# DoubangoTelecom/compv

Measured on AMD Instinct MI355X. Metric: Mpixels/s Sobel->Canny->HoughSHT on 4K uint8, higher is better.
Workload: dtype u8; 1 GPU; batched 3840x2160 uint8 frames, Sobel3x3 -> Canny(59,119) -> HoughSHT(rho=1, theta=1deg, thr=100); 256 distinct frames resident per GPU as 8 batches of 32, a step processes one batch, steps rotate over the batches; frames_per_gpu=32, resident_batches=8, parallelism=frames sharded across 1 GPU(s), no data-path collective

## Files before the change

### compv_amd/csrc/api.cpp

```cpp
#include "api_internal.hpp"

namespace {
__attribute__((noinline, optnone)) float libmCosf(float x) { return cosf(x); }
__attribute__((noinline, optnone)) float libmSinf(float x) { return sinf(x); }

void gradientThresholds(float fLow, float fHigh, int* tLow, int* tHigh)
{
	const float l = fLow < 1.f ? 1.f : (fLow > 65535.f ? 65535.f : fLow);
	const float h = fHigh < 1.f ? 1.f : (fHigh > 65535.f ? 65535.f : fHigh);
	uint16_t lo = static_cast<uint16_t>(l), hi = static_cast<uint16_t>(h);
	lo = static_cast<uint16_t>(std::max<int>(1, lo));
	hi = static_cast<uint16_t>(std::max<int>(lo + 2, hi));
	*tLow = lo; *tHigh = hi;
}

void cannyCoverage(size_t W, int* simdEnd, int* cStart)
{
	const size_t maxCols = W - 1;
	size_t mpw = 1;
	if (maxCols >= 16) mpw = 16; else if (maxCols >= 8) mpw = 8;
	if (mpw == 1) { *simdEnd = 1; *cStart = 1; return; }
	size_t col = 1;
	while (col + (mpw - 1) < maxCols) col += mpw;
	*simdEnd = static_cast<int>(col);
// ... 550 lines not shown
	if (run.copyBack) HIPCHK(ctx, hipMemcpyAsync(run.copyBack, run.patchOut, bytes, hipMemcpyDeviceToDevice, st));
	p->bitsValid = true;
	return COMPVHIP_OK;
}

int compvhip_plan_canny(compvhip_plan* p, const uint8_t* d_in, float tLow, float tHigh, int ksize, int type, uint8_t* d_edges, void* stream)
{
	if (!p) return COMPVHIP_E_INVALID_PARAMETER;
	if (int rc = refuseBeyondLaunchLimit(p->ctx, p->frames, "compvhip_plan_canny")) return rc;
	StepRun run;
	return planCannyImpl(p, run, d_in, tLow, tHigh, ksize, type, d_edges, static_cast<hipStream_t>(stream), true);
}

int compvhip_api::pixfmtBytes(int fmt)
{
	if (fmt < COMPVHIP_FMT_RGBA32 || fmt > COMPVHIP_FMT_Y) return 0;
	return fmt <= COMPVHIP_FMT_BGRA32 ? 4 : (fmt <= COMPVHIP_FMT_BGR24 ? 3 : (fmt == COMPVHIP_FMT_Y ? 1 : 2));
}

int compvhip_api::checkPixfmt(compvhip_ctx* ctx, int fmt, size_t W)
{
	if (fmt > COMPVHIP_FMT_Y && fmt <= COMPVHIP_FMT_HSV) return fail(ctx, COMPVHIP_E_INVALID_PARAMETER, "a format of the colour conversion calls only (compvhip_convert_frames)");
	if (!pixfmtBytes(fmt)) return fail(ctx, COMPVHIP_E_NOT_IMPLEMENTED, "pixel format without a grayscale conversion");
	if ((fmt == COMPVHIP_FMT_YUYV422 || fmt == COMPVHIP_FMT_UYVY422) && (W & 1)) return fail(ctx, COMPVHIP_E_INVALID_PARAMETER, "packed 4:2:2 needs an even width");
	return COMPVHIP_OK;
}

int compvhip_plan_grayscale(compvhip_plan* p, const uint8_t* d_in, int pixfmt, uint8_t* d_gray, void* stream)
{
	if (!p) return COMPVHIP_E_INVALID_PARAMETER;
	compvhip_ctx* ctx = p->ctx;
	if (!d_in || !d_gray) return fail(ctx, COMPVHIP_E_INVALID_PARAMETER, "null frame pointer");
	const int rc = checkPixfmt(ctx, pixfmt, p->W);
	if (rc) return rc;
	HIPCHK(ctx, hipSetDevice(ctx->device));
	hipStream_t st = static_cast<hipStream_t>(stream);
	if (p->timing) timelineClear(p);
	GrayArgs a;
	a.in = d_in; a.out = d_gray; a.W = static_cast<int>(p->W); a.H = static_cast<int>(p->H); a.S = static_cast<int>(p->S); a.So = static_cast<int>(p->S);
	Stamp s(p, st, "gray_kernel");
	HIPCHK(ctx, launch_gray(a, pixfmt, static_cast<int>(p->frames), st));
	return COMPVHIP_OK;
}

int compvhip_plan_otsu(compvhip_plan* p, const uint8_t* d_gray, int32_t* d_thresholds, void* stream)
{
	if (!p) return COMPVHIP_E_INVALID_PARAMETER;
	compvhip_ctx* ctx = p->ctx;
	if (!d_gray || !d_thresholds) return fail(ctx, COMPVHIP_E_INVALID_PARAMETER, "null pointer");
	if (misaligned(3, d_thresholds)) return fail(ctx, COMPVHIP_E_INVALID_PARAMETER, "levels must be 4-byte aligned");
	HIPCHK(ctx, hipSetDevice(ctx->device));
	int rc = ensurePreproc(p);
	if (rc) return rc;
	hipStream_t st = static_cast<hipStream_t>(stream);
	if (p->timing) timelineClear(p);
	Stamp s(p, st, "otsu_kernels");
	HIPCHK(ctx, launch_otsu(d_gray, static_cast<int>(p->W), static_cast<int>(p->H), static_cast<int>(p->S), p->S * p->H, static_cast<int>(p->frames), 0.5f, 1.f,
	                        p->hist, d_thresholds, nullptr, st));
	return COMPVHIP_OK;
}

int compvhip_api::checkFxpKernel(compvhip_ctx* ctx, size_t W, size_t H, const uint16_t* vt, const uint16_t* hz, size_t k)
{
	if (!vt || !hz || !(k & 1) || W < k || H < k) return fail(ctx, COMPVHIP_E_INVALID_PARAMETER, "convolution kernel: null, even size or larger than the image");
	if (k < 3 || k > static_cast<size_t>(kFxpMaxTaps)) return fail(ctx, COMPVHIP_E_NOT_IMPLEMENTED, "fixed-point convolution supports kernel sizes 3..15");
	return COMPVHIP_OK;
}

int compvhip_plan_convlt1_fixedpoint(compvhip_plan* p, const uint8_t* d_in, const uint16_t* vtKern, const uint16_t* hzKern, size_t kernSize, uint8_t* d_out,
                                     void* stream)
{
	if (!p) return COMPVHIP_E_INVALID_PARAMETER;
	compvhip_ctx* ctx = p->ctx;
	if (!d_in || !d_out) return fail(ctx, COMPVHIP_E_INVALID_PARAMETER, "null frame pointer");
	int rc = refuseBeyondLaunchLimit(ctx, p->frames, "compvhip_plan_convlt1_fixedpoint");
	if (rc) return rc;
	rc = checkFxpKernel(ctx, p->W, p->H, vtKern, hzKern, kernSize);
	if (rc) return rc;
	HIPCHK(ctx, hipSetDevice(ctx->device));
	const size_t span = p->S * p->H * p->frames;
	const bool alias = overlaps(d_in, span, d_out, span);
	if (alias) HIPCHK(ctx, p->blurTmp.reserve(ctx, span));
	hipStream_t st = static_cast<hipStream_t>(stream);
	if (p->timing) timelineClear(p);
	Stamp s(p, st, "convlt_fxp_kernels");
	HIPCHK(ctx, launch_convlt_fxp(d_in, p->blurTmp, d_out, static_cast<int>(p->W), static_cast<int>(p->H), static_cast<int>(p->S), p->S * p->H,
	                              static_cast<int>(p->frames), vtKern, hzKern, static_cast<int>(kernSize), st));
	return COMPVHIP_OK;
}

int compvhip_plan_edge_dete(compvhip_plan* p, const uint8_t* d_in, int op, uint8_t* d_out, void* stream)
{
	if (!p) return COMPVHIP_E_INVALID_PARAMETER;
	compvhip_ctx* ctx = p->ctx;
	if (!d_in || !d_out) return fail(ctx, COMPVHIP_E_INVALID_PARAMETER, "null frame pointer");
	if (op != COMPVHIP_OP_SOBEL && op != COMPVHIP_OP_SCHARR && op != COMPVHIP_OP_PREWITT)
		return fail(ctx, COMPVHIP_E_INVALID_PARAMETER, "invalid detector id");
	const size_t bytes = p->S * p->H * p->frames;
	if (overlaps(d_in, bytes, d_out, bytes)) return fail(ctx, COMPVHIP_E_INVALID_PARAMETER, "d_in and d_out must not alias");
	HIPCHK(ctx, hipSetDevice(ctx->device));
	hipStream_t st = static_cast<hipStream_t>(stream);
	if (p->timing) timelineClear(p);
	EdgeDeteArgs a;
	a.in = d_in; a.out = d_out; a.gmax = p->sums;
	a.inFrameStride = p->S * p->H; a.outFrameStride = p->S * p->H;
	a.W = static_cast<int>(p->W); a.H = static_cast<int>(p->H); a.S = static_cast<int>(p->S); a.So = static_cast<int>(p->S);
	a.tilesX = p->tilesX; a.tilesY = p->tilesY;
	Stamp s(p, st, "edge_dete_kernels");
	HIPCHK(ctx, launch_edge_dete(a, op, static_cast<int>(p->frames), st));
	return COMPVHIP_OK;
}

int compvhip_api::planShtImpl(compvhip_plan* p, const uint8_t* d_edges, int threshold, int maxLines, compvhip_line* d_lines, size_t lineCap, int32_t* d_counts,
                              hipStream_t st, const ShtOpts& o)
{
	compvhip_ctx* ctx = p->ctx;
	if (threshold <= 0) return fail(ctx, COMPVHIP_E_INVALID_PARAMETER, "threshold must be > 0");
	if (misaligned(3, d_lines, d_counts)) return fail(ctx, COMPVHIP_E_INVALID_PARAMETER, "lines and counts must be 4-byte aligned");
	if (!d_edges && !p->bitsValid) return fail(ctx, COMPVHIP_E_INVALID_STATE, "no edge masks: run compvhip_plan_canny first or pass d_edges");
	HIPCHK(ctx, hipSetDevice(ctx->device));
	int rc = ensureSht(p);
	if (rc) return rc;
	rc = ensureLineCap(p, std::max(lineCap, kMinLineCap));
	if (rc) return rc;
	if (p->timing && o.clearTimeline) timelineClear(p);
	const int frames = static_cast<int>(p->frames);
	size_t sortN = o.sortN;
	if (d_edges) {
		Stamp s(p, st, "bytes_to_bits_kernel");
		HIPCHK(ctx, launch_bytes_to_bits(d_edges, static_cast<int>(p->W), static_cast<int>(p->H), static_cast<int>(p->S), p->S * p->H, p->ebits, p->wb,
		                                 p->bitsFrameStride, frames, st));
		p->bitsValid = false;
	}
	ShtArgs a = shtArgs(p, threshold);
	a.outCounts = d_counts;
	a.hostStep = o.hostSlot; a.stepFlags = p->flags;
	const size_t capAll = p->lineCap * p->frames;
	const bool deviceSort = p->deviceSort && !o.pairsOnly;
	if (sortN != kSortExact) sortN = std::min(sortN, capAll);
	a.sortN = (o.pairsOnly || deviceSort || sortN == kSortExact) ? 0 : sortN;
	if (!p->countersFresh) HIPCHK(ctx, hipMemsetAsync(p->counters, 0, sizeof(int) * p->nCounts, st));
	p->countersFresh = false;
	{ Stamp s(p, st, "sht_compact_kernel"); HIPCHK(ctx, launch_sht_compact_tiles(a, p->vt, frames, st)); }
	{ Stamp s(p, st, "sht_vote_kernel"); HIPCHK(ctx, launch_sht_vote_tiles(a, p->vt, frames, st)); }
	{ Stamp s(p, st, "sht_reduce_kernel"); HIPCHK(ctx, launch_sht_reduce_tiles(a, p->vt, frames, st)); }
	{ Stamp s(p, st, "sht_lines_kernel"); HIPCHK(ctx, launch_sht_lines(a, frames, st)); }
	if (o.pairsOnly) {
		return COMPVHIP_OK;
	}
	if (deviceSort) {
		if (d_lines && lineCap) {
			Stamp s(p, st, "sht_sort_lines");
			ShtSortArgs q;
			q.sortedKeys = p->keysB; q.sortedVals = p->valsB; q.chunkHist = p->chunkHist; q.strengthStart = p->strengthStart; q.chunks = p->sortChunks;
			HIPCHK(ctx, launch_sht_sort_lines(a, q, frames, p->thetaStep, maxLines, d_lines, lineCap, st));
		}
		return COMPVHIP_OK;
	}
	if (sortN == kSortExact) {
		HIPCHK(ctx, hipMemcpyAsync(p->hTotals, p->lineTotal, sizeof(unsigned int), hipMemcpyDeviceToHost, st));
		HIPCHK(ctx, hipStreamSynchronize(st));
		sortN = std::min(static_cast<size_t>(p->hTotals[0]), capAll);
	}
	if (sortN) {
		Stamp s(p, st, "sht_sort_lines");
		size_t tb = p->sortTempBytes;
		hipError_t e = sht_sort_pairs(p->sortTemp, tb, p->keysA, p->keysB, p->valsA, p->valsB, sortN, p->keyBits, st);
		if (e != hipSuccess) return fail(ctx, COMPVHIP_E_HIP, "radix sort", e);
	}
	if (d_lines && lineCap) {
		Stamp s(p, st, "sht_decode_kernel");
		HIPCHK(ctx, launch_sht_decode(p->keysB, p->valsB, p->lineCounts, p->lineCap, frames, static_cast<int>(p->T), static_cast<int>(p->W + p->H), p->thetaStep, maxLines,
		                              p->strengthBits, d_lines, lineCap, st));
	}
	return COMPVHIP_OK;
}

int compvhip_plan_houghsht(compvhip_plan* p, const uint8_t* d_edges, int threshold, int maxLines, compvhip_line* d_lines, size_t lineCap,
                           int32_t* d_counts, void* stream)
{
	if (!p) return COMPVHIP_E_INVALID_PARAMETER;
	if (int rc = refuseBeyondLaunchLimit(p->ctx, p->frames, "compvhip_plan_houghsht")) return rc;
	return planShtImpl(p, d_edges, threshold, maxLines, d_lines, lineCap, d_counts, static_cast<hipStream_t>(stream), ShtOpts());
}

static int checkStep(compvhip_plan* p, const StepParams& sp)
{
	compvhip_ctx* ctx = p->ctx;
	int rc = refuseBeyondLaunchLimit(ctx, p->frames, "compvhip_plan_pipeline");
	if (rc) return rc;
	if (!sp.d_in || !sp.d_edges) return fail(ctx, COMPVHIP_E_INVALID_PARAMETER, "null frame pointer");
	rc = checkPixfmt(ctx, sp.pixfmt, p->W);
	if (rc) return rc;
	if (sp.d_cart && (!sp.d_lines || !sp.d_counts)) return fail(ctx, COMPVHIP_E_INVALID_PARAMETER, "toCartesian needs the line and count buffers");
	if (misaligned(3, sp.d_lines, sp.d_counts, sp.d_otsu, sp.d_cart)) return fail(ctx, COMPVHIP_E_INVALID_PARAMETER, "lines, counts, levels and endpoints must be 4-byte aligned");
	return COMPVHIP_OK;
}

static int enqueueStep(compvhip_plan* p, StepRun& run, const StepParams& sp, hipStream_t st, bool clearTimeline)
{
	compvhip_ctx* ctx = p->ctx;
	HIPCHK(ctx, hipSetDevice(ctx->device));
	const uint8_t* luma = sp.d_in;
	if (sp.pixfmt != COMPVHIP_FMT_Y) {
		uint8_t* gray = sp.d_gray;
		if (!gray) {
			HIPCHK(ctx, p->grayTmp.reserve(ctx, p->S * p->H * p->frames));
			gray = p->grayTmp;
		}
		if (p->timing && clearTimeline) timelineClear(p);
		clearTimeline = false;
		GrayArgs a;
		a.in = sp.d_in; a.out = gray; a.W = static_cast<int>(p->W); a.H = static_cast<int>(p->H); a.S = static_cast<int>(p->S); a.So = static_cast<int>(p->S);
		Stamp s(p, st, "gray_kernel");
		HIPCHK(ctx, launch_gray(a, sp.pixfmt, static_cast<int>(p->frames), st));
		luma = gray;
	}
	int rc = planCannyImpl(p, run, luma, sp.tLow, sp.tHigh, sp.ksize, sp.thresholdType, sp.d_edges, st, false, clearTimeline);
	if (rc) return rc;
	if (sp.d_otsu && sp.thresholdType == COMPVHIP_CANNY_THRESHOLD_OTSU)
		HIPCHK(ctx, hipMemcpyAsync(sp.d_otsu, p->otsu, sizeof(int32_t) * p->frames, hipMemcpyDeviceToDevice, st));
	return COMPVHIP_OK;
}

static int toCartesianImpl(compvhip_plan* p, const compvhip_line* d_lines, const int32_t* d_counts, size_t lineCap, int maxLines, float* d_cart, void* stream);

static int enqueueStepTail(compvhip_plan* p, const StepRun& run, const StepParams& sp, hipStream_t st, size_t sortN)
{
	ShtOpts o;
	o.clearTimeline = false; o.sortN = sortN; o.hostSlot = run.hostSlot;
	int rc = planShtImpl(p, nullptr, sp.threshold, sp.maxLines, sp.d_lines, sp.lineCap, sp.d_counts, st, o);
	if (rc) return rc;
	if (sp.d_cart) {
		rc = toCartesianImpl(p, sp.d_lines, sp.d_counts, sp.lineCap, sp.maxLines, sp.d_cart, st);
		if (rc) return rc;
	}
	return COMPVHIP_OK;
}

static int runStepSync(compvhip_plan* p, const StepParams& sp, hipStream_t st)
{
	StepRun run;
	int rc = enqueueStep(p, run, sp, st, true);
	if (rc) return rc;
	const size_t bytes = p->S * p->H * p->frames;
	for (;;) {
		rc = enqueueStepTail(p, run, sp, st, kSortExact);
		if (rc) return rc;
		bool done = false;
		rc = resolveConverged(p, run, st, &done);
		if (rc) return rc;
		if (done) break;
		do {
			rc = enqueueResolve(p, run, kSpecRounds, st);
			if (rc) return rc;
			rc = resolveConverged(p, run, st, &done);
			if (rc) return rc;
		} while (!done);
		if (run.copyBack) HIPCHK(p->ctx, hipMemcpyAsync(run.copyBack, run.patchOut, bytes, hipMemcpyDeviceToDevice, st));
	}
	return COMPVHIP_OK;
}

static int runStepAsync(compvhip_plan* p, const StepParams& sp, hipStream_t st, int* ticket)
{
	compvhip_ctx* ctx = p->ctx;
	*ticket = -1;
	int slot = -1;
	for (int i = 0; i < kAsyncDepth; ++i) if (!p->steps[i].used) { slot = i; break; }
	if (slot < 0) return fail(ctx, COMPVHIP_E_INVALID_STATE, "too many steps in flight: call compvhip_plan_wait first");
	const size_t bytes = p->S * p->H * p->frames;
	const size_t inBytes = bytes * static_cast<size_t>(sp.pixfmt == COMPVHIP_FMT_Y ? 1 : pixfmtBytes(sp.pixfmt));
	if (overlaps(sp.d_in, inBytes, sp.d_edges, bytes))
		return fail(ctx, COMPVHIP_E_INVALID_PARAMETER, "the asynchronous step needs distinct input and edge buffers");
	compvhip_plan::AsyncStep& stp = p->steps[slot];
	HIPCHK(ctx, hipSetDevice(ctx->device));
	if (!stp.done) HIPCHK(ctx, hipEventCreateWithFlags(&stp.done, hipEventDisableTiming));
	if (p->timeline.size() > kMaxTimeline) timelineClear(p);
	int* slotHost = p->hRounds + kSlotStride * slot;
	slotHost[kSlotTotal] = ~0;
	for (int i = 0; i < 4; ++i) slotHost[kSlotFlags + i] = 1;
	StepRun run;
	run.hostSlot = p->hRoundsDev + kSlotStride * slot;
	int rc = enqueueStep(p, run, sp, st, false);
	if (rc) return rc;
	rc = ensureSht(p);
	if (rc) return rc;
	rc = ensureLineCap(p, std::max(sp.lineCap, kMinLineCap));
	if (rc) return rc;
	const size_t capAll = p->lineCap * p->frames;
	const size_t sortN = p->deviceSort ? capAll : asyncSortRange(p->recentTotals, capAll);
	static_assert(kMaxRounds >= 4 && kSpecRounds <= 4, "the round flags compvhip_plan_wait looks at");
	if (run.roundsUsed > 4) return fail(ctx, COMPVHIP_E_INVALID_STATE, "more speculative rounds than flags the step reports");
	rc = enqueueStepTail(p, run, sp, st, sortN);
	if (rc) return rc;
	HIPCHK(ctx, hipEventRecord(stp.done, st));
	stp.used = true; stp.replay = false; stp.seq = ++p->stepSeq; stp.stream = st; stp.sp = sp; stp.sortN = sortN; stp.rounds = run.roundsUsed;
	*ticket = slot;
	return COMPVHIP_OK;
}

static StepParams classicStep(const uint8_t* d_in, float tLow, float tHigh, int threshold, int maxLines, uint8_t* d_edges, compvhip_line* d_lines, size_t lineCap,
                              int32_t* d_counts)
{
	StepParams sp;
	sp.d_in = d_in; sp.tLow = tLow; sp.tHigh = tHigh; sp.threshold = threshold; sp.maxLines = maxLines; sp.d_edges = d_edges; sp.d_lines = d_lines;
	sp.lineCap = lineCap; sp.d_counts = d_counts;
// ... 115 lines not shown
```

### compv_amd/csrc/kernels.hpp

```cpp
#pragma once
#include <hip/hip_runtime.h>
#include <stddef.h>
#include <stdint.h>

#include "../../include/compv_hip.h"

namespace compvhip {

#ifndef COMPVHIP_BAND_H
#define COMPVHIP_BAND_H 64
#endif
constexpr int kBandH = COMPVHIP_BAND_H;
#ifndef COMPVHIP_BAND_WORDS
#define COMPVHIP_BAND_WORDS 64
#endif
constexpr int kBandWords = COMPVHIP_BAND_WORDS;
constexpr int kResolveThreads = 512;
constexpr int kFrameSlot = 32;
constexpr int kResolveRows = kBandH * kBandWords / kResolveThreads;

struct CannyArgs {
	const uint8_t* in;
	uint8_t* out;
	uint32_t* ebits;
	uint32_t* ubits;
	const int2* thrDev;
	size_t inFrameStride, outFrameStride, bitsFrameStride;
	int W, H, S, So;
	int wb;
	int tilesX, tilesY;
	int tLow, tHigh;
	int simdEnd, cStart;
	int blockRows, groups;
	int ksize;
	int* zero; int nZero;
};

struct ResolveArgs {
	uint32_t* ebits;
	uint32_t* ubits;
	uint8_t* out;
	int* flags;
	uint8_t* dirty;
	size_t outFrameStride, bitsFrameStride;
	int H, So, wb;
	int round;
};

hipError_t launch_canny_tiles(const CannyArgs& a, int frames, bool gap, hipStream_t stream);
hipError_t launch_canny_tiles_swar(const CannyArgs& a, int frames, bool gap, hipStream_t stream);
hipError_t launch_canny_resolve(const ResolveArgs& a, int frames, hipStream_t stream);
size_t canny_resolve_dirty_bytes(int H, int wb, int frames);
hipError_t launch_mean_thresholds(const uint8_t* in, int W, int H, int S, size_t frameStride, int frames, float fLow, float fHigh,
                                  unsigned int* sums, int2* thr, hipStream_t stream);

struct EdgeDeteArgs {
	const uint8_t* in;
	uint8_t* out;
	unsigned int* gmax;
	size_t inFrameStride, outFrameStride;
	int W, H, S, So;
	int tilesX, tilesY;
	int blockRows, groups;
};
hipError_t launch_edge_dete(const EdgeDeteArgs& a, int op, int frames, hipStream_t stream);

struct ConvertArgs {
	const uint8_t* in[3];
	uint8_t* out[3];
	size_t inRow[3], inFrame[3], outRow[3], outFrame[3];
	int W, H;
};
hipError_t launch_convert(const ConvertArgs& a, int inFmt, int outFmt, int frames, hipStream_t stream);

struct GrayArgs {
	const uint8_t* in;
	uint8_t* out;
	int W, H, S, So;
};
hipError_t launch_gray(const GrayArgs& a, int fmt, int frames, hipStream_t stream);
constexpr int kOtsuMaxChunks = 128;
hipError_t launch_otsu(const uint8_t* in, int W, int H, int S, size_t frameStride, int frames, float fLowFactor, float fHighFactor, uint32_t* hist,
                       int32_t* otsu, void* thr, hipStream_t stream);

constexpr int kFxpMaxTaps = 15;
struct FxpArgs {
	const uint8_t* in;
	uint8_t* out;
	size_t inFrameStride, outFrameStride;
	int W, H, S, So;
	uint32_t kern[kFxpMaxTaps];
};
hipError_t launch_convlt_fxp(const uint8_t* in, uint8_t* tmp, uint8_t* out, int W, int H, int S, size_t frameStride, int frames, const uint16_t* vtKern,
                             const uint16_t* hzKern, int K, hipStream_t stream);

struct I16Args {
	const void* in;
	int16_t* out;
	int W, H, S, So, K;
	int kern[kFxpMaxTaps];
};
hipError_t launch_convlt_i16(const void* in, bool inIsU8, int16_t* tmp, int16_t* out, int W, int H, int S, int So, const int16_t* vtKern, const int16_t* hzKern,
                             int K, hipStream_t stream);

struct ShtArgs {
	const uint32_t* ebits;
	uint32_t* edges;
	int* edgeCounts;
	uint16_t* acc;
	const int32_t* sinQ;
	const int32_t* cosQ;
	uint32_t* lineKeys;
	uint32_t* lineVals;
	uint8_t* nmsFlags;
	int nmsRows;
	int* blockCounts;
	int lineBlocks;
	const int2* nmsRange;
	int nmsGroups;
	int* lineCounts;
	const int* stepFlags;
	int* hostStep;
	int32_t* outCounts;
	int* frameTotals;
	unsigned int* lineTotal;
	size_t sortN;
	size_t bitsFrameStride, edgeCap, accFrameStride, lineCap;
	int W, H, wb;
	int R, T, accPitch, barrier;
	int threshold, nmsLastCol;
	int frames;
	int strengthBits;
};
struct ShtTileArgs {
	const int32_t* kt;
	const int32_t* rowBase;
	uint8_t* partLo;
	uint8_t* partHi;
	uint8_t* colFlag;
	const int2* reach;
	int* tileCounts;
	int nx, ny, TW, TH, tiles;
	int Rw, rwPitch;
	int Tpad, groups;
	size_t tileCap;
};
constexpr int kShtMaxWindow = 1264;
hipError_t launch_sht_compact_tiles(const ShtArgs& a, const ShtTileArgs& v, int frames, hipStream_t stream);
hipError_t launch_sht_vote_tiles(const ShtArgs& a, const ShtTileArgs& v, int frames, hipStream_t stream);
hipError_t launch_sht_reduce_tiles(const ShtArgs& a, const ShtTileArgs& v, int frames, hipStream_t stream);
hipError_t launch_bytes_to_bits(const uint8_t* edges, int W, int H, int S, size_t frameStride, uint32_t* ebits, int wb, size_t bitsFrameStride,
                                int frames, hipStream_t stream);
hipError_t launch_sht_lines(const ShtArgs& a, int frames, hipStream_t stream);
hipError_t launch_sht_decode(const uint32_t* keys, const uint32_t* vals, const int* counts, size_t lineCap, int frames, int T, int barrier, float thetaStep,
                             int maxLines, int strengthBits, void* lines , size_t outCap, hipStream_t stream);
int sht_nms_groups(int T);
size_t sht_nms_rows(int R);
int sht_lines_blocks(int R);
hipError_t launch_sht_cartesian(const void* lines , const int* counts, size_t lineCap, int maxLines, int frames, int T, const float* cosT,
                                const float* invSinT, float thetaStep, float widthF, float r, float* out , hipStream_t stream);
hipError_t launch_sht_acc_transpose(const uint16_t* accT, int R, int T, int accPitch, int32_t* out, size_t outStride, hipStream_t stream);
constexpr int kShtSortChunk = 4096;
constexpr int kShtSortMaxStrengthBits = 13;
constexpr int kShtSortMaxChunks = 32;
struct ShtSortArgs {
	uint32_t* sortedKeys;
	uint32_t* sortedVals;
	uint16_t* chunkHist;
	uint32_t* strengthStart;
	int chunks;
};
hipError_t launch_sht_sort_lines(const ShtArgs& a, const ShtSortArgs& q, int frames, float thetaStep, int maxLines, void* lines , size_t outCap,
                                 hipStream_t stream);
hipError_t sht_sort_pairs(void* temp, size_t& tempBytes, const uint32_t* keysIn, uint32_t* keysOut, const uint32_t* valsIn, uint32_t* valsOut, size_t n,
                          int keyBits, hipStream_t stream);

struct ShtLineSetArgs {
	const uint32_t* ebits;
	const uint8_t* edges;
	size_t bitsFrameStride, edgeFrameStride;
	int wb, S;
	const int32_t* sinQ;
	const int32_t* cosQ;
	const compvhip_line* lines;
	const int32_t* lineCounts;
	size_t lineCap;
	int nLines;
	int W, H, R, T, barrier;
};
struct ShtSegArgs : ShtLineSetArgs {
	int minLength, maxGap;
	int32_t* perLine;
	compvhip_segment* segs;
	size_t segCap;
	int32_t* segCounts;
	int frame0;
};
hipError_t launch_sht_segments(const ShtSegArgs& a, int frames, int phase, hipStream_t stream);

struct ShtFitArgs : ShtLineSetArgs {
	int halfWidth;
	const compvhip_segment* segs;
	const int32_t* segCounts;
	size_t segCap;
	compvhip_line_fit* fits;
	size_t fitCap;
	int32_t* fitCounts;
	compvhip_line* refined;
	int frame0;
};
static_assert(sizeof(ShtLineSetArgs) == 104 && sizeof(ShtSegArgs) == 152 && sizeof(ShtFitArgs) == 176, "kernel argument layout");
hipError_t launch_sht_fit(const ShtFitArgs& a, int frames, hipStream_t stream);

struct CompArgs {
	const uint32_t* bits;
	size_t bitsFrameStride;
	int wb;
	int W, H;
	int words;
	uint32_t lastMask;
	int conn8;
	int minPixels;
	int32_t* parent;
	size_t parentFrameStride;
	int ps;
	int wantLabels;
	compvhip_component* comps;
	size_t compCap;
	int32_t* compCounts;
	int32_t* rowCounts;
	int frame0;
};
hipError_t launch_components(const CompArgs& a, int frames, int phase, hipStream_t stream);

struct ThreshArgs {
	const uint8_t* in;
	uint8_t* out;
	const int32_t* levels;
	size_t frameStride;
	int W, H, S;
	int t8;
};
hipError_t launch_threshold(const ThreshArgs& a, int frames, hipStream_t stream);
struct AdaptArgs {
	const uint8_t* in;
	uint8_t* out;
	size_t frameStride;
	int W, H, S;
	int r;
	uint32_t k;
	int delta, maxVal, invert;
};
hipError_t launch_threshold_adaptive(const AdaptArgs& a, int frames, hipStream_t stream);
constexpr int kMorphMaxStrel = 31;
constexpr size_t kMorphGeneralMaxMembers = 15;
enum { kMorphGeneral = 0, kMorphRect = 1, kMorphCross = 2 };
struct MorphArgs {
	const uint8_t* in;
	uint8_t* out;
	size_t frameStride;
	int W, H, S;
	int sw, sh;
	int dilate;
	int replicate;
	int kind;
	uint32_t rows[kMorphMaxStrel];
};
hipError_t launch_morph(const MorphArgs& a, int frames, hipStream_t stream);

struct FastArgs {
	const uint8_t* in;
	uint8_t* scores;
	size_t frameStride;
	int W, H, S;
	int t, N, nonmax;
	int maxFeatures;
	int* rowCounts;
	int* rowOffsets;
	int* hist;
	int* minScore;
	compvhip_corner* corners; size_t cornerCap;
	int32_t* counts;
};
hipError_t launch_fast(const FastArgs& a, int frames, int stage, hipStream_t stream);

constexpr int kMatchQueryBlock = 256;
constexpr int kMatchTrainSlice = 128;
constexpr int kMatchMaxKnn = 8;
constexpr int kMatchMaxDwords = 32;
struct MatchSliceArgs {
	const uint8_t* query;
	const uint8_t* train;
	const int32_t* queryCounts; const int32_t* trainCounts;
	int queryCap, trainCap, queryStride, trainStride;
	int queryShared, trainShared;
	int descDwords;
	int knn;
	int slices;
	uint32_t* partial;
	compvhip_match* matches;
};
hipError_t launch_match_slices(const MatchSliceArgs& a, int pairs, hipStream_t stream);
hipError_t launch_match_merge(const MatchSliceArgs& a, int pairs, hipStream_t stream);
hipError_t launch_match_reference(const MatchSliceArgs& a, int pairs, hipStream_t stream);
struct MatchGoodArgs {
	const compvhip_match* matches;
	const compvhip_match* reverse;
	const int32_t* queryCounts; const int32_t* trainCounts;
	int queryCap, trainCap, trainShared, knn;
	double ratio; int maxDistance, crossCheck;
	compvhip_match* good; size_t goodCap;
	int32_t* counts;
};
hipError_t launch_match_good(const MatchGoodArgs& a, int pairs, hipStream_t stream);

constexpr int kHomographySolveBlock = 64;
constexpr int kHomographyScoreBlock = 256;
struct HomographyPointsArgs {
	const compvhip_match* good; int goodCap;
	const int32_t* goodCounts;
// ... 232 lines not shown
```

### compv_amd/csrc/sht_sort_kernels.hip

```cpp
#include "device.hpp"

#include <type_traits>

namespace compvhip {

namespace {

constexpr int kChunk = kShtSortChunk;
constexpr int kSortThreads = 1024;
constexpr int kBins = 1 << kShtSortMaxStrengthBits;
static_assert(kChunk == 4096 && kBins == 8192, "key layout: 13 bits of inverted strength above 12 bits of chunk position");

}

__global__ __launch_bounds__(kSortThreads) void sht_chunk_sort_kernel(ShtArgs a, ShtSortArgs q)
{
	__shared__ uint32_t s_key[kChunk];
	__shared__ uint32_t s_hist[kBins];
	__shared__ uint32_t s_cnt[kSortThreads], s_wsum[kSortThreads / 64];
	__shared__ unsigned long long s_part[kSortThreads / 64];
	const int frame = blockIdx.y, chunk = blockIdx.x, t = threadIdx.x;
	const size_t nf = min((size_t)max(a.lineCounts[frame], 0), a.lineCap);
	const size_t c0 = (size_t)chunk * kChunk;
	if (c0 >= nf) return;
	const int m = (int)min((size_t)kChunk, nf - c0);
	const size_t base = dense_frame_base<kSortThreads>(a.lineCounts, frame, a.lineCap, s_part) + c0;
	const uint32_t mask = (1u << a.strengthBits) - 1u;
	const uint32_t* __restrict__ kin = a.lineKeys + base;
	const uint32_t* __restrict__ vin = a.lineVals + base;
	uint32_t e[4];
	{
		uint32_t kraw[4];
#pragma unroll
		for (int u = 0; u < 4; ++u) kraw[u] = kin[min(u * kSortThreads + t, m - 1)];
		asm volatile("" : "+v"(kraw[0]), "+v"(kraw[1]), "+v"(kraw[2]), "+v"(kraw[3]));
#pragma unroll
		for (int u = 0; u < 4; ++u) {
			const int i = u * kSortThreads + t;
			e[u] = i < m ? (((mask - (kraw[u] & mask)) << 12) | (uint32_t)i) : 0xffffffffu;
		}
	}
#pragma unroll
	for (int u = 0; u < kBins / kSortThreads; ++u) s_hist[t + u * kSortThreads] = 0u;
	const int lane = t & 63, wave = t >> 6;
	auto radix_pass = [&](auto nbits, int shift) {
		constexpr int NB = decltype(nbits)::value, BINS = 1 << NB;
		s_cnt[t] = 0u;
		__syncthreads();
		uint32_t rank[4], slot[4];
#pragma unroll
		for (int u = 0; u < 4; ++u) {
			const uint32_t d = (e[u] >> shift) & (uint32_t)(BINS - 1);
			uint64_t same = ~0ull;
#pragma unroll
			for (int b = 0; b < NB; ++b) {
				const bool bit = (d >> b) & 1u;
				const uint64_t bal = __ballot(bit);
				same &= bit ? bal : ~bal;
			}
			rank[u] = __builtin_amdgcn_mbcnt_hi((uint32_t)(same >> 32), __builtin_amdgcn_mbcnt_lo((uint32_t)same, 0u));
			slot[u] = (d * 4u + (uint32_t)u) * (uint32_t)(kSortThreads / 64) + (uint32_t)wave;
			if (rank[u] == 0u) s_cnt[slot[u]] = (uint32_t)__popcll(same);
		}
		__syncthreads();
		const uint32_t c = s_cnt[t];
		const uint32_t incl = wave_incl_scan(c, lane);
		if (lane == 63) s_wsum[wave] = incl;
		__syncthreads();
		uint32_t before = 0;
#pragma unroll
		for (int w = 0; w < kSortThreads / 64; ++w) before += (w < wave) ? s_wsum[w] : 0u;
		s_cnt[t] = before + incl - c;
		__syncthreads();
#pragma unroll
		for (int u = 0; u < 4; ++u) s_key[s_cnt[slot[u]] + rank[u]] = e[u];
		__syncthreads();
#pragma unroll
		for (int u = 0; u < 4; ++u) e[u] = s_key[u * kSortThreads + t];
	};
	radix_pass(std::integral_constant<int, 4>{}, 12);
	radix_pass(std::integral_constant<int, 3>{}, 16);
	radix_pass(std::integral_constant<int, 3>{}, 19);
	radix_pass(std::integral_constant<int, 3>{}, 22);
	uint32_t* __restrict__ kout = q.sortedKeys + base;
	uint32_t* __restrict__ vout = q.sortedVals + base;
	{
		uint32_t kk[4]; int lo[4], hi[4];
#pragma unroll
		for (int u = 0; u < 4; ++u) { const int i = min(t + u * kSortThreads, m - 1); kk[u] = s_key[i]; lo[u] = 0; hi[u] = i; }
#pragma unroll
		for (int s = 0; s < 12; ++s) {
#pragma unroll
			for (int u = 0; u < 4; ++u) {
				const int mid = (lo[u] + hi[u]) >> 1;
				const bool ge = s_key[mid] >= (kk[u] & ~4095u);
				hi[u] = ge ? mid : hi[u];
				lo[u] = ge ? lo[u] : mid + 1;
			}
		}
		uint32_t cell[4];
#pragma unroll
		for (int u = 0; u < 4; ++u) cell[u] = vin[kk[u] & 4095u];
		asm volatile("" : "+v"(cell[0]), "+v"(cell[1]), "+v"(cell[2]), "+v"(cell[3]));
#pragma unroll
		for (int u = 0; u < 4; ++u) {
			const int i = t + u * kSortThreads;
			if (i < m) {
				kout[i] = (kk[u] & ~4095u) | (uint32_t)(i - lo[u]);
				vout[i] = cell[u];
				atomicAdd(&s_hist[kk[u] >> 12], 1u);
			}
		}
	}
	__syncthreads();
	uint4* __restrict__ hout = reinterpret_cast<uint4*>(q.chunkHist + ((size_t)frame * q.chunks + chunk) * kBins);
	{
		const uint32_t* h = s_hist + 8 * t;
		hout[t] = make_uint4(h[0] | (h[1] << 16), h[2] | (h[3] << 16), h[4] | (h[5] << 16), h[6] | (h[7] << 16));
	}
}

__global__ __launch_bounds__(kSortThreads) void sht_strength_scan_kernel(ShtArgs a, ShtSortArgs q)
{
	__shared__ uint32_t s_wave[kSortThreads / 64];
	const int frame = blockIdx.x, t = threadIdx.x;
	const size_t nf = min((size_t)max(a.lineCounts[frame], 0), a.lineCap);
	if (nf == 0) return;
	const int nch = (int)((nf + kChunk - 1) / kChunk);
	uint32_t tot[8] = { 0, 0, 0, 0, 0, 0, 0, 0 };
	const uint4* __restrict__ h = reinterpret_cast<const uint4*>(q.chunkHist + (size_t)frame * q.chunks * kBins) + t;
	auto add8 = [](uint32_t (&d)[8], const uint4& v) {
		d[0] += v.x & 0xffffu; d[1] += v.x >> 16; d[2] += v.y & 0xffffu; d[3] += v.y >> 16;
		d[4] += v.z & 0xffffu; d[5] += v.z >> 16; d[6] += v.w & 0xffffu; d[7] += v.w >> 16;
	};
	const uint4 zero4 = make_uint4(0u, 0u, 0u, 0u);
	for (int c0 = 0; c0 < nch; c0 += 4) {
		uint4 v[4];
#pragma unroll
		for (int u = 0; u < 4; ++u) v[u] = h[(size_t)min(c0 + u, nch - 1) * (kBins / 8)];
#pragma unroll
		for (int u = 0; u < 4; ++u) add8(tot, (c0 + u < nch) ? v[u] : zero4);
	}
	uint32_t sum = 0;
#pragma unroll
	for (int u = 0; u < 8; ++u) { const uint32_t c = tot[u]; tot[u] = sum; sum += c; }
	uint32_t incl = sum;
	const int lane = t & 63, wave = t >> 6;
#pragma unroll
	for (int o = 1; o < 64; o <<= 1) {
		const uint32_t n = __shfl_up(incl, o);
		if (lane >= o) incl += n;
	}
	if (lane == 63) s_wave[wave] = incl;
	__syncthreads();
	uint32_t before = 0;
#pragma unroll
	for (int w = 0; w < kSortThreads / 64; ++w) before += (w < wave) ? s_wave[w] : 0u;
	const uint32_t excl = before + incl - sum;
	uint4* __restrict__ out = reinterpret_cast<uint4*>(q.strengthStart + (size_t)frame * kBins) + 2 * t;
	out[0] = make_uint4(excl + tot[0], excl + tot[1], excl + tot[2], excl + tot[3]);
	out[1] = make_uint4(excl + tot[4], excl + tot[5], excl + tot[6], excl + tot[7]);
}

__global__ __launch_bounds__(256) void sht_place_lines_kernel(ShtArgs a, ShtSortArgs q, float thetaStep, int maxLines, compvhip_line* __restrict__ lines, size_t outCap)
{
	__shared__ unsigned long long s_part[4];
	const int frame = blockIdx.y;
	const size_t nf = min((size_t)max(a.lineCounts[frame], 0), a.lineCap);
	const size_t i0 = (size_t)blockIdx.x * 256;
	if (i0 >= nf) return;
	const size_t base = dense_frame_base<256>(a.lineCounts, frame, a.lineCap, s_part);
	const size_t i = i0 + threadIdx.x;
	if (i >= nf) return;
	size_t limit = nf;
	if (maxLines > 0 && limit > (size_t)maxLines) limit = (size_t)maxLines;
	if (limit > outCap) limit = outCap;
	const uint32_t kv = q.sortedKeys[base + i];
	const uint32_t inv = kv >> 12, rank = kv & 4095u;
	const int c = (int)(i >> 12);
	size_t pos = (size_t)q.strengthStart[(size_t)frame * kBins + inv] + rank;
	const uint16_t* __restrict__ h = q.chunkHist + (size_t)frame * q.chunks * kBins + inv;
	for (int c0 = 0; c0 < c; c0 += 4) {
		uint32_t v[4];
#pragma unroll
		for (int u = 0; u < 4; ++u) v[u] = h[(size_t)min(c0 + u, c) * kBins];
#pragma unroll
		for (int u = 0; u < 4; ++u) pos += (c0 + u < c) ? v[u] : 0u;
	}
	if (pos >= limit) return;
	const uint32_t cell = q.sortedVals[base + i];
	const int row = (int)(cell / (uint32_t)a.T), col = (int)(cell - (uint32_t)row * (uint32_t)a.T);
	compvhip_line o;
	o.rho = (float)(a.barrier - row);
	o.theta = __fmul_rn((float)col, thetaStep);
	o.strength = (int32_t)(((1u << a.strengthBits) - 1u) - inv);
	o.row = row; o.col = col;
	lines[(size_t)frame * outCap + pos] = o;
}

hipError_t launch_sht_sort_lines(const ShtArgs& a, const ShtSortArgs& q, int frames, float thetaStep, int maxLines, void* lines, size_t outCap, hipStream_t stream)
{
	if (!lines || !outCap) return hipSuccess;
	hipLaunchKernelGGL(sht_chunk_sort_kernel, dim3((unsigned)q.chunks, (unsigned)frames), dim3(kSortThreads), 0, stream, a, q);
	hipLaunchKernelGGL(sht_strength_scan_kernel, dim3((unsigned)frames), dim3(kSortThreads), 0, stream, a, q);
	hipLaunchKernelGGL(sht_place_lines_kernel, dim3((unsigned)(q.chunks * (kChunk / 256)), (unsigned)frames), dim3(256), 0, stream, a, q, thetaStep, maxLines,
	                   reinterpret_cast<compvhip_line*>(lines), outCap);
	return hipGetLastError();
}

}
```

Baseline: 426,700 Mpixels/s.

## Replace per-chunk radix sort with stable ballot-based rank counting

The per-chunk LDS radix sort (four passes plus a binary search and a value gather) becomes a ranking kernel. Each wave groups lanes that share a strength via bit ballots, and waves commit packed u16 counters to LDS in turn order, which gives each line a stable rank within its strength. The placement kernel then reads values straight from the unsorted input. Chunk size doubles to 8192 and the LDS counter footprint scales with strengthBits. This removes the sorted-values buffer and most of the shuffling work, at the cost of serialising the waves' commits.

```diff
diff --git a/compv_amd/csrc/api.cpp b/compv_amd/csrc/api.cpp
--- a/compv_amd/csrc/api.cpp
+++ b/compv_amd/csrc/api.cpp
@@ -726,7 +726,7 @@
 		if (d_lines && lineCap) {
 			Stamp s(p, st, "sht_sort_lines");
 			ShtSortArgs q;
-			q.sortedKeys = p->keysB; q.sortedVals = p->valsB; q.chunkHist = p->chunkHist; q.strengthStart = p->strengthStart; q.chunks = p->sortChunks;
+			q.rankKeys = p->keysB; q.chunkHist = p->chunkHist; q.strengthStart = p->strengthStart; q.chunks = p->sortChunks;
 			HIPCHK(ctx, launch_sht_sort_lines(a, q, frames, p->thetaStep, maxLines, d_lines, lineCap, st));
 		}
 		return COMPVHIP_OK;
diff --git a/compv_amd/csrc/kernels.hpp b/compv_amd/csrc/kernels.hpp
--- a/compv_amd/csrc/kernels.hpp
+++ b/compv_amd/csrc/kernels.hpp
@@ -160,12 +160,11 @@
 hipError_t launch_sht_cartesian(const void* lines , const int* counts, size_t lineCap, int maxLines, int frames, int T, const float* cosT,
                                 const float* invSinT, float thetaStep, float widthF, float r, float* out , hipStream_t stream);
 hipError_t launch_sht_acc_transpose(const uint16_t* accT, int R, int T, int accPitch, int32_t* out, size_t outStride, hipStream_t stream);
-constexpr int kShtSortChunk = 4096;
+constexpr int kShtSortChunk = 8192;
 constexpr int kShtSortMaxStrengthBits = 13;
-constexpr int kShtSortMaxChunks = 32;
+constexpr int kShtSortMaxChunks = 16;
 struct ShtSortArgs {
-	uint32_t* sortedKeys;
-	uint32_t* sortedVals;
+	uint32_t* rankKeys;
 	uint16_t* chunkHist;
 	uint32_t* strengthStart;
 	int chunks;
diff --git a/compv_amd/csrc/sht_sort_kernels.hip b/compv_amd/csrc/sht_sort_kernels.hip
--- a/compv_amd/csrc/sht_sort_kernels.hip
+++ b/compv_amd/csrc/sht_sort_kernels.hip
@@ -1,123 +1,102 @@
 #include "device.hpp"
 
-#include <type_traits>
+#include <algorithm>
 
 namespace compvhip {
 
 namespace {
 
 constexpr int kChunk = kShtSortChunk;
+constexpr int kChunkBits = __builtin_ctz(kChunk);
+constexpr int kChunkRows = kChunk / 64;
+constexpr int kRankWaves = 16;
 constexpr int kSortThreads = 1024;
 constexpr int kBins = 1 << kShtSortMaxStrengthBits;
-static_assert(kChunk == 4096 && kBins == 8192, "key layout: 13 bits of inverted strength above 12 bits of chunk position");
+static_assert(kChunk == 1 << kChunkBits && kShtSortMaxStrengthBits + kChunkBits <= 32, "rank word: the inverted strength above the rank");
+static_assert(kBins == 8 * kSortThreads, "the scan kernel's thread owns 8 strengths");
+static_assert(kChunk < 65536, "a chunk's histogram is u16");
+static_assert(kChunkRows % kRankWaves == 0 && kRankWaves <= 16, "whole rows per wave; dense_frame_base's partial sums have 16 slots");
 
 }
 
-__global__ __launch_bounds__(kSortThreads) void sht_chunk_sort_kernel(ShtArgs a, ShtSortArgs q)
+__global__ __launch_bounds__(kRankWaves * 64) void sht_chunk_rank_kernel(ShtArgs a, ShtSortArgs q)
 {
-	__shared__ uint32_t s_key[kChunk];
-	__shared__ uint32_t s_hist[kBins];
-	__shared__ uint32_t s_cnt[kSortThreads], s_wsum[kSortThreads / 64];
-	__shared__ unsigned long long s_part[kSortThreads / 64];
+	constexpr int THREADS = kRankWaves * 64, B = kChunkRows / kRankWaves;
+	extern __shared__ __attribute__((aligned(16))) uint32_t s_rank[];
+	unsigned long long* s_part = reinterpret_cast<unsigned long long*>(s_rank);
+	uint32_t* s_idle = s_rank + 32;
+	uint32_t* s_cnt = s_rank + 96;
 	const int frame = blockIdx.y, chunk = blockIdx.x, t = threadIdx.x;
 	const size_t nf = min((size_t)max(a.lineCounts[frame], 0), a.lineCap);
 	const size_t c0 = (size_t)chunk * kChunk;
 	if (c0 >= nf) return;
 	const int m = (int)min((size_t)kChunk, nf - c0);
-	const size_t base = dense_frame_base<kSortThreads>(a.lineCounts, frame, a.lineCap, s_part) + c0;
-	const uint32_t mask = (1u << a.strengthBits) - 1u;
+	const int lane = t & 63, wave = t >> 6;
+	const int bits = a.strengthBits;
+	const uint32_t mask = (1u << bits) - 1u;
+	const int words = max((1 << bits) >> 1, 4);
+	for (int w = t; w < words; w += THREADS) s_cnt[w] = 0u;
+	const size_t base = dense_frame_base<THREADS>(a.lineCounts, frame, a.lineCap, s_part) + c0;
 	const uint32_t* __restrict__ kin = a.lineKeys + base;
-	const uint32_t* __restrict__ vin = a.lineVals + base;
-	uint32_t e[4];
-	{
-		uint32_t kraw[4];
+	uint32_t* __restrict__ kout = q.rankKeys + base;
+	const int row0 = wave * B;
+
+	struct Row { uint32_t inv, rank, size; int first; bool valid; };
+	auto load_rows = [&](uint32_t (&k)[B], int r0) {
 #pragma unroll
-		for (int u = 0; u < 4; ++u) kraw[u] = kin[min(u * kSortThreads + t, m - 1)];
-		asm volatile("" : "+v"(kraw[0]), "+v"(kraw[1]), "+v"(kraw[2]), "+v"(kraw[3]));
+		for (int j = 0; j < B; ++j) k[j] = kin[min((r0 + j) * 64 + lane, m - 1)];
+	};
+	auto ballot_rows = [&](const uint32_t (&k)[B], int r0, Row (&row)[B]) {
+		uint64_t same[B];
 #pragma unroll
-		for (int u = 0; u < 4; ++u) {
-			const int i = u * kSortThreads + t;
-			e[u] = i < m ? (((mask - (kraw[u] & mask)) << 12) | (uint32_t)i) : 0xffffffffu;
+		for (int j = 0; j < B; ++j) {
+			row[j].valid = (r0 + j) * 64 + lane < m;
+			row[j].inv = mask - (k[j] & mask);
+			same[j] = __ballot(row[j].valid);
 		}
-	}
+		for (int b = 0; b < bits; ++b) {
 #pragma unroll
-	for (int u = 0; u < kBins / kSortThreads; ++u) s_hist[t + u * kSortThreads] = 0u;
-	const int lane = t & 63, wave = t >> 6;
-	auto radix_pass = [&](auto nbits, int shift) {
-		constexpr int NB = decltype(nbits)::value, BINS = 1 << NB;
-		s_cnt[t] = 0u;
-		__syncthreads();
-		uint32_t rank[4], slot[4];
-#pragma unroll
-		for (int u = 0; u < 4; ++u) {
-			const uint32_t d = (e[u] >> shift) & (uint32_t)(BINS - 1);
-			uint64_t same = ~0ull;
-#pragma unroll
-			for (int b = 0; b < NB; ++b) {
-				const bool bit = (d >> b) & 1u;
+			for (int j = 0; j < B; ++j) {
+				const bool bit = (row[j].inv >> b) & 1u;
 				const uint64_t bal = __ballot(bit);
-				same &= bit ? bal : ~bal;
-			}
-			rank[u] = __builtin_amdgcn_mbcnt_hi((uint32_t)(same >> 32), __builtin_amdgcn_mbcnt_lo((uint32_t)same, 0u));
-			slot[u] = (d * 4u + (uint32_t)u) * (uint32_t)(kSortThreads / 64) + (uint32_t)wave;
-			if (rank[u] == 0u) s_cnt[slot[u]] = (uint32_t)__popcll(same);
-		}
-		__syncthreads();
-		const uint32_t c = s_cnt[t];
-		const uint32_t incl = wave_incl_scan(c, lane);
-		if (lane == 63) s_wsum[wave] = incl;
-		__syncthreads();
-		uint32_t before = 0;
-#pragma unroll
-		for (int w = 0; w < kSortThreads / 64; ++w) before += (w < wave) ? s_wsum[w] : 0u;
-		s_cnt[t] = before + incl - c;
-		__syncthreads();
-#pragma unroll
-		for (int u = 0; u < 4; ++u) s_key[s_cnt[slot[u]] + rank[u]] = e[u];
-		__syncthreads();
-#pragma unroll
-		for (int u = 0; u < 4; ++u) e[u] = s_key[u * kSortThreads + t];
-	};
-	radix_pass(std::integral_constant<int, 4>{}, 12);
-	radix_pass(std::integral_constant<int, 3>{}, 16);
-	radix_pass(std::integral_constant<int, 3>{}, 19);
-	radix_pass(std::integral_constant<int, 3>{}, 22);
-	uint32_t* __restrict__ kout = q.sortedKeys + base;
-	uint32_t* __restrict__ vout = q.sortedVals + base;
-	{
-		uint32_t kk[4]; int lo[4], hi[4];
-#pragma unroll
-		for (int u = 0; u < 4; ++u) { const int i = min(t + u * kSortThreads, m - 1); kk[u] = s_key[i]; lo[u] = 0; hi[u] = i; }
-#pragma unroll
-		for (int s = 0; s < 12; ++s) {
-#pragma unroll
-			for (int u = 0; u < 4; ++u) {
-				const int mid = (lo[u] + hi[u]) >> 1;
-				const bool ge = s_key[mid] >= (kk[u] & ~4095u);
-				hi[u] = ge ? mid : hi[u];
-				lo[u] = ge ? lo[u] : mid + 1;
+				same[j] &= bit ? bal : ~bal;
 			}
 		}
-		uint32_t cell[4];
 #pragma unroll
-		for (int u = 0; u < 4; ++u) cell[u] = vin[kk[u] & 4095u];
-		asm volatile("" : "+v"(cell[0]), "+v"(cell[1]), "+v"(cell[2]), "+v"(cell[3]));
+		for (int j = 0; j < B; ++j) {
+			row[j].rank = __builtin_amdgcn_mbcnt_hi((uint32_t)(same[j] >> 32), __builtin_amdgcn_mbcnt_lo((uint32_t)same[j], 0u));
+			row[j].size = (uint32_t)__popcll(same[j]);
+			row[j].first = __ffsll((unsigned long long)same[j]) - 1;
+		}
+	};
+	auto commit_rows = [&](const Row (&row)[B], uint32_t (&old)[B]) {
 #pragma unroll
-		for (int u = 0; u < 4; ++u) {
-			const int i = t + u * kSortThreads;
-			if (i < m) {
-				kout[i] = (kk[u] & ~4095u) | (uint32_t)(i - lo[u]);
-				vout[i] = cell[u];
-				atomicAdd(&s_hist[kk[u] >> 12], 1u);
-			}
+		for (int j = 0; j < B; ++j) {
+			const bool first = row[j].valid && row[j].rank == 0u;
+			old[j] = atomicAdd(first ? &s_cnt[row[j].inv >> 1] : &s_idle[lane], first ? row[j].size << ((row[j].inv & 1u) << 4) : 0u);
 		}
+	};
+	auto store_rows = [&](int r0, const Row (&row)[B], const uint32_t (&old)[B]) {
+#pragma unroll
+		for (int j = 0; j < B; ++j) {
+			const uint32_t before = (__shfl(old[j], row[j].first) >> ((row[j].inv & 1u) << 4)) & 0xffffu;
+			if (row[j].valid) kout[(r0 + j) * 64 + lane] = (row[j].inv << kChunkBits) | (before + row[j].rank);
+		}
+	};
+
+	uint32_t k[B], old[B];
+	Row row[B];
+	load_rows(k, row0);
+	ballot_rows(k, row0, row);
+	const int turns = (m + B * 64 - 1) / (B * 64);
+	for (int turn = 0; turn < turns; ++turn) {
+		if (wave == turn) commit_rows(row, old);
+		__syncthreads();
 	}
-	__syncthreads();
+	if (wave < turns) store_rows(row0, row, old);
 	uint4* __restrict__ hout = reinterpret_cast<uint4*>(q.chunkHist + ((size_t)frame * q.chunks + chunk) * kBins);
-	{
-		const uint32_t* h = s_hist + 8 * t;
-		hout[t] = make_uint4(h[0] | (h[1] << 16), h[2] | (h[3] << 16), h[4] | (h[5] << 16), h[6] | (h[7] << 16));
-	}
+	const uint4* cnt4 = reinterpret_cast<const uint4*>(s_cnt);
+	for (int v = t; v < kBins / 8; v += THREADS) hout[v] = 4 * v < words ? cnt4[v] : make_uint4(0u, 0u, 0u, 0u);
 }
 
 __global__ __launch_bounds__(kSortThreads) void sht_strength_scan_kernel(ShtArgs a, ShtSortArgs q)
@@ -175,9 +154,10 @@
 	size_t limit = nf;
 	if (maxLines > 0 && limit > (size_t)maxLines) limit = (size_t)maxLines;
 	if (limit > outCap) limit = outCap;
-	const uint32_t kv = q.sortedKeys[base + i];
-	const uint32_t inv = kv >> 12, rank = kv & 4095u;
-	const int c = (int)(i >> 12);
+	const uint32_t kv = q.rankKeys[base + i];
+	const uint32_t cell = a.lineVals[base + i];
+	const uint32_t inv = kv >> kChunkBits, rank = kv & (uint32_t)(kChunk - 1);
+	const int c = (int)(i >> kChunkBits);
 	size_t pos = (size_t)q.strengthStart[(size_t)frame * kBins + inv] + rank;
 	const uint16_t* __restrict__ h = q.chunkHist + (size_t)frame * q.chunks * kBins + inv;
 	for (int c0 = 0; c0 < c; c0 += 4) {
@@ -188,7 +168,6 @@
 		for (int u = 0; u < 4; ++u) pos += (c0 + u < c) ? v[u] : 0u;
 	}
 	if (pos >= limit) return;
-	const uint32_t cell = q.sortedVals[base + i];
 	const int row = (int)(cell / (uint32_t)a.T), col = (int)(cell - (uint32_t)row * (uint32_t)a.T);
 	compvhip_line o;
 	o.rho = (float)(a.barrier - row);
@@ -201,7 +180,8 @@
 hipError_t launch_sht_sort_lines(const ShtArgs& a, const ShtSortArgs& q, int frames, float thetaStep, int maxLines, void* lines, size_t outCap, hipStream_t stream)
 {
 	if (!lines || !outCap) return hipSuccess;
-	hipLaunchKernelGGL(sht_chunk_sort_kernel, dim3((unsigned)q.chunks, (unsigned)frames), dim3(kSortThreads), 0, stream, a, q);
+	const size_t rankLds = 384 + sizeof(uint32_t) * (size_t)std::max((1 << a.strengthBits) >> 1, 4);
+	hipLaunchKernelGGL(sht_chunk_rank_kernel, dim3((unsigned)q.chunks, (unsigned)frames), dim3(kRankWaves * 64), rankLds, stream, a, q);
 	hipLaunchKernelGGL(sht_strength_scan_kernel, dim3((unsigned)frames), dim3(kSortThreads), 0, stream, a, q);
 	hipLaunchKernelGGL(sht_place_lines_kernel, dim3((unsigned)(q.chunks * (kChunk / 256)), (unsigned)frames), dim3(256), 0, stream, a, q, thetaStep, maxLines,
 	                   reinterpret_cast<compvhip_line*>(lines), outCap);
```

Result: faster. 436,700 Mpixels/s (median of 6 runs) (+2.4%).
